# princeton-vl/CER-MVS

Measured on AMD Instinct MI355X. Metric: depth-maps/sec (ref+N src views) at DTU 1600x1184; HBM GB/s vs roofline, higher is better.
Workload: dtype f32 [dense convs: f32 operands split into 2 x f16, f32 accumulate; encoders f16 main term + the two 2^-11 correction terms in e2m3 (FP6, one power-of-two scale per 16-channel block: features 4e-5 from the three-term form), update-block convs f16 main term + the two 2^-11 correction terms in e4m3 on

## Files before the change

### cer-mvs_amd/csrc/conv_s16.hip

```cpp
#include "conv_s16_shared.hpp"
#include "pack.hpp"

struct SxStage {
    int kind;
    const char* base;
    long mtb;
    int g;
};

template <int WM_, int WN_, int MT, int EPI, int F8>
__global__ __launch_bounds__(256, 2) void conv3x3_s16_kernel(const S16Args a) {
    constexpr int TH = WM_ * 2 * MT, HR = TH + 2;
    constexpr int ABUF = HR * (F8 ? SX_ROWB8 : SX_ROWB);
    constexpr int NPIX = HR * SX_HW, NITEM = NPIX * 4, ITEMS = (NITEM + 255) / 256;
    constexpr bool F6 = F8 == 2;
    constexpr int NITEM8 = NPIX * 4, ITEMS8 = F8 ? (NITEM8 + 255) / 256 : 1;
    constexpr int NB = WN_ * 32;
    constexpr int DROWS = HR + 6;
    extern __shared__ __attribute__((aligned(16))) char sx_smem[];
    float* ldsD = reinterpret_cast<float*>(sx_smem + 2 * ABUF);

    const int tid = threadIdx.x, lane = tid & 63, wave = __builtin_amdgcn_readfirstlane(tid >> 6);
    const int wm = wave / WN_, wn = wave % WN_;
    const int li = lane & 31, kg = lane >> 5;
    CER_FUZZ_INIT();
#if SX_TRACE
    unsigned long long trace_t[24];
    int trace_n = 0;
    trace_t[trace_n++] = __builtin_readcyclecounter();
#define SX_STAMP() do { if (trace_n < 24) trace_t[trace_n++] = __builtin_readcyclecounter(); } while (0)
#else
#define SX_STAMP() do { } while (0)
#endif

    auto xcd_order = [](int n, int j) {
        const int q = n >> 3, r = n & 7, xcd = j & 7, k = j >> 3;
        return (xcd < r ? xcd * (q + 1) : r * (q + 1) + (xcd - r) * q) + k;
    };
    int tile, by;
    int tile_y, tile_x;
    if (a.border_first) {
        const int bid = blockIdx.x, tys = a.ntiles / a.tiles_x, nbord = 2 * tys + 2 * (a.tiles_x - 2);
        if (bid < 2 * tys) {
            tile_y = bid >> 1; tile_x = (bid & 1) ? a.tiles_x - 1 : 0;
        } else if (bid < nbord) {
            const int r2 = bid - 2 * tys;
            tile_y = (r2 & 1) ? tys - 1 : 0; tile_x = 1 + (r2 >> 1);
        } else {
            const int i = xcd_order(a.ntiles - nbord, bid - nbord);
            tile_y = 1 + i / (a.tiles_x - 2); tile_x = 1 + i - (tile_y - 1) * (a.tiles_x - 2);
        }
        tile = tile_y * a.tiles_x + tile_x;
        by = 0;
    } else {
        const int vid = xcd_order((int)gridDim.x, (int)blockIdx.x);
        tile = vid / a.ny; by = vid - tile * a.ny;
        tile_y = tile / a.tiles_x; tile_x = tile - tile_y * a.tiles_x;
    }
    const int ty0 = tile_y * TH, tx0 = tile_x * SX_TW;
    const int nb0 = by * NB;
    const int NT = a.cout >> 5;

    int ntens = a.nsrc;
    const float* dsrc = nullptr;
    if (a.kind[a.nsrc - 1] == 1) { ntens = a.nsrc - 1; dsrc = reinterpret_cast<const float*>(a.src[a.nsrc - 1]); }
    const bool interior = ty0 >= 1 && ty0 + TH <= a.h - 1 && tx0 >= 1 && tx0 + SX_TW <= a.w - 1;
    const bool coll = dsrc && a.wpk_c && (interior || a.edge);
    int nsteps = 0;
    for (int s = 0; s < ntens; ++s) nsteps += (a.ch[s] >> 4) * 9;
    const int nsteps_t = nsteps;
    if (dsrc) nsteps += coll ? 6 : 36;
#if SX_STAGGER
    if ((int)gridDim.x > 3 * SX_STAGGER_CUS && (int)blockIdx.x < 2 * SX_STAGGER_CUS) {
        const unsigned hw = __builtin_amdgcn_s_getreg((4 << 0) | (0 << 6) | (31 << 11));
        if ((hw >> SX_STAGGER_BIT) & 1)
            for (int i = 0; i < nsteps * SX_STAGGER; ++i) __builtin_amdgcn_s_sleep(1);
    }
#endif
    const char* wlane = reinterpret_cast<const char*>(coll ? a.wpk_c : a.wpk) + ((long)(nb0 >> 5) + wn) * 2048 + lane * 16;
    const long wstep = (long)NT * 2048;
    const char* wlane8 = reinterpret_cast<const char*>(coll ? a.wpk_c : a.wpk) + ((long)(nb0 >> 5) + wn) * 4096 + lane * 16;

    int xh[3], xl[3];
#pragma unroll
    for (int dx = 0; dx < 3; ++dx) {
        const int col = (li & 15) + dx;
        const int base = (2 * wm * MT + (li >> 4)) * SX_ROWB + col * 64;
        const int sl = kg ^ ((col >> 2) & 3);
        xh[dx] = base + sl * 16;
        xl[dx] = base + (sl ^ 2) * 16;
    }

    int st_pk[ITEMS];
#pragma unroll
    for (int i = 0; i < ITEMS; ++i) {
        const int it = tid + 256 * i;
        const int n = min(it >> 2, NPIX - 1), ps = it & 3;
        const int r = n / SX_HW, c = n - r * SX_HW;
        const int gy = ty0 + r - 1, gx = tx0 + c - 1;
        const bool valid = gy >= 0 && gy < a.h && gx >= 0 && gx < a.w;
        const int cy = min(max(gy, 0), a.h - 1), cx = min(max(gx, 0), a.w - 1);
        const int logical = ps ^ ((c >> 2) & 3);
        st_pk[i] = ((cy >> 1) * a.mtx + (cx >> 4)) | ((((cy & 1) << 4) | (cx & 15)) << 20) | (logical << 25) | ((valid ? 1 : 0) << 27) |
                   ((it < NITEM ? 1 : 0) << 28);
    }
    constexpr int IB = (ITEMS + 1) / 2;
    uint4 raw[IB];
    int vary = 0;
    auto stage_load = [&](const SxStage& st, int batch) {
#pragma unroll
        for (int k = 0; k < IB; ++k) {
            const int i = batch * IB + k;
            if (i >= ITEMS) break;
            const int pk = st_pk[i] ^ vary;
            const char* p = st.base + (long)(pk & 0xFFFFF) * st.mtb + (((pk >> 25) & 3) * 512 + ((pk >> 20) & 31) * 16);
            raw[k] = *reinterpret_cast<const uint4*>(p);
        }
    };
    auto stage_store = [&](int bufoff, int batch) {
        CER_FUZZ_POINT();
        const int tid_ = tid ^ vary;
#pragma unroll
        for (int k = 0; k < IB; ++k) {
            const int i = batch * IB + k;
            if (i >= ITEMS) break;
            const int pk = st_pk[i] ^ vary;
            const unsigned m = (pk & (1 << 27)) ? 0xFFFFFFFFu : 0u;
            uint4 v = raw[k];
            v.x &= m; v.y &= m; v.z &= m; v.w &= m;
            const int it = tid_ + 256 * i;
            const int n = it >> 2, r = n / SX_HW, c = n - r * SX_HW;
            if (pk & (1 << 28)) *reinterpret_cast<uint4*>(sx_smem + bufoff + (r * SX_PITCH + c) * 64 + (it & 3) * 16) = v;
        }
    };
    int xa[3];
    if constexpr (F8) {
#pragma unroll
        for (int dx = 0; dx < 3; ++dx) {
            const int col = (li & 15) + dx;
            xa[dx] = (2 * wm * MT + (li >> 4)) * SX_ROWB8 + col * 128 + (((2 * kg) ^ ((col >> 1) & 7)) << 4);
        }
    }
    int st8_pk[ITEMS8];
    if constexpr (F8) {
#pragma unroll
        for (int i = 0; i < ITEMS8; ++i) {
            const int it = tid + 256 * i;
            const int n = min(it >> 2, NPIX - 1);
            const int r = n / SX_HW, c = n - r * SX_HW;
            const int gy = ty0 + r - 1, gx = tx0 + c - 1;
            const bool valid = gy >= 0 && gy < a.h && gx >= 0 && gx < a.w;
            const int cy = min(max(gy, 0), a.h - 1), cx = min(max(gx, 0), a.w - 1);
            st8_pk[i] = ((cy >> 1) * a.mtx + (cx >> 4)) | ((((cy & 1) << 4) | (cx & 15)) << 20) | ((valid ? 1 : 0) << 28) | ((it < NITEM8 ? 1 : 0) << 29);
        }
    }
    constexpr int IB8 = (ITEMS8 + 2) / 3;
    constexpr int NLD8 = 2;
    uint4 raw8[IB8][NLD8];
    auto stage8_addr = [&](const SxStage& st, int pk, int it) {
        return st.base + (long)(pk & 0xFFFFF) * st.mtb + (((it >> 1) & 1) * 2048 + (it & 1) * 512 + ((pk >> 20) & 31) * 16);
    };
    auto stage6_put = [&](int bufoff, int pk, int it, uint4 vh, uint4 vl) {
        const unsigned m = (pk & (1 << 28)) ? 0xFFFFFFFFu : 0u;
        vh.x &= m; vh.y &= m; vh.z &= m; vh.w &= m;
// ... 98 lines not shown
                const float u[8] = {v[8 * kh], v[8 * kh + 1], v[8 * kh + 2], v[8 * kh + 3], v[8 * kh + 4], v[8 * kh + 5], v[8 * kh + 6], v[8 * kh + 7]};
                half8 hi, lo;
                sx_split8(u, a.disp_scale, hi, lo);
                *reinterpret_cast<half8*>(px + ((kh ^ key) * 16)) = hi;
                SX_LDS_STORE_WAIT();
                *reinterpret_cast<half8*>(px + (((2 + kh) ^ key) * 16)) = lo;
                SX_LDS_STORE_WAIT();
            }
        }
    };
    auto gen_collapsed = [&](int g, int bufoff) {
        auto half_unit = [&](auto kh_tag, int n) {
            constexpr int kh = decltype(kh_tag)::value;
            const int pr = n >> 4, pc = n & 15;
            const float* dp = ldsD + pr * SX_DTW + pc;
            const float ctr = dp[4 * SX_DTW + 4];
            float v[8];
#pragma unroll
            for (int k = 0; k < 8; ++k) {
                const int s = 16 * g + 8 * kh + k;
                const int sy = (s * 57) >> 9, sx = s - 9 * sy;
                v[k] = (s < 81) ? 100.0f * (dp[sy * SX_DTW + sx] - ctr) : 0.f;
            }
            const int c = pc + 1;
            char* px = sx_smem + bufoff + ((pr + 1) * SX_PITCH + c) * 64;
            const int key = (c >> 2) & 3;
            half8 hi, lo;
            sx_split8(v, a.disp_scale, hi, lo);
            *reinterpret_cast<half8*>(px + ((kh ^ key) * 16)) = hi;
            SX_LDS_STORE_WAIT();
            *reinterpret_cast<half8*>(px + (((2 + kh) ^ key) * 16)) = lo;
            SX_LDS_STORE_WAIT();
        };
        CER_FUZZ_POINT();
        for (int u = tid ^ vary; u < TH * SX_TW; u += 256) {
            half_unit(std::integral_constant<int, 0>{}, u);
            half_unit(std::integral_constant<int, 1>{}, u);
        }
    };
    auto stage_tap = [&](const SxStage& st, int bufoff, int t) {
        if (st.kind == 2) {
            if constexpr (F8) {
                if (t == 0) stage8_load(st, 0);
                if (t == 2) { stage8_store(bufoff, 0); stage8_load(st, 1); }
                if (t == 4) { stage8_store(bufoff, 1); stage8_load(st, 2); }
                if (t == 6) stage8_store(bufoff, 2);
            } else {
                if (t == 0) stage_load(st, 0);
                if (t == 3) { stage_store(bufoff, 0); stage_load(st, 1); }
                if (t == 6) stage_store(bufoff, 1);
            }
        } else if (t == 6) {
            if (st.kind == 1) gen_literal(st.g, bufoff);
            else if (st.kind == 3) gen_collapsed(st.g, bufoff);
        }
    };
    auto barrier = [&]() {
        __builtin_amdgcn_fence(__ATOMIC_RELEASE, "workgroup", "local");
        __builtin_amdgcn_s_barrier();
        __builtin_amdgcn_fence(__ATOMIC_ACQUIRE, "workgroup", "local");
        CER_FUZZ_POINT();
    };

    int ngroups_t = 0;
    for (int s = 0; s < ntens; ++s) ngroups_t += a.ch[s] >> (F8 ? 5 : 4);
    const int ngroups = ngroups_t + (dsrc ? (coll ? 6 : 4) : 0);
    auto describe = [&](int gi) {
        SxStage st;
        st.kind = 0; st.base = nullptr; st.mtb = 0; st.g = 0;
        if (gi >= ngroups) return st;
        if (gi >= ngroups_t) { st.kind = coll ? 3 : 1; st.g = gi - ngroups_t; return st; }
        int s = 0, g = gi;
        while (g >= (a.ch[s] >> (F8 ? 5 : 4))) { g -= a.ch[s] >> (F8 ? 5 : 4); ++s; }
        st.kind = 2; st.base = a.src[s] + g * (F8 ? 4096 : 2048); st.mtb = (long)(a.ch[s] >> 4) * 2048;
        return st;
    };

    struct XFrag { half8 h[MT], l[MT]; };
    struct WFrag { half8 h, l; };
    XFrag fx;
    WFrag fw[3];
    auto load_w = [&](WFrag& f, int step) {
        const char* p = wlane + (long)min(step, nsteps - 1) * wstep;
        f.h = *reinterpret_cast<const half8*>(p);
        f.l = *reinterpret_cast<const half8*>(p + 1024);
    };
    const SxStage st0 = describe(0);
    uint4 raw0[F8 ? NLD8 * ITEMS8 : ITEMS];
    if (st0.kind == 2) {
        if constexpr (F8) {
#pragma unroll
            for (int i = 0; i < ITEMS8; ++i) {
                const char* p = stage8_addr(st0, st8_pk[i], tid + 256 * i);
#pragma unroll
                for (int q = 0; q < NLD8; ++q) raw0[NLD8 * i + q] = *reinterpret_cast<const uint4*>(p + 1024 * q);
            }
        } else {
#pragma unroll
            for (int i = 0; i < ITEMS; ++i) {
                const int pk = st_pk[i];
                raw0[i] = *reinterpret_cast<const uint4*>(st0.base + (long)(pk & 0xFFFFF) * st0.mtb + (((pk >> 25) & 3) * 512 + ((pk >> 20) & 31) * 16));
            }
        }
    }
    constexpr int DITEMS = (DROWS * SX_DTW + 255) / 256;
    float dval[DITEMS];
    if (dsrc) {
#pragma unroll
        for (int i = 0; i < DITEMS; ++i) {
            const int idx = tid + 256 * i;
            const int r = idx / SX_DTW, c = idx - r * SX_DTW;
            const int gy = ty0 + r - 4, gx = tx0 + c - 4;
            dval[i] = (idx < DROWS * SX_DTW && gy >= 0 && gy < a.h && gx >= 0 && gx < a.w) ? dsrc[(long)gy * a.w + gx] : 0.f;
        }
    }
    typedef unsigned uintx3 __attribute__((ext_vector_type(3)));
    struct Op8 {
        uint4 a;
        typename std::conditional<F8 == 2, uintx3, uint4>::type b;
        __device__ __forceinline__ void load(const char* p0, const char* p1) {
            a = *reinterpret_cast<const uint4*>(p0);
            b = *reinterpret_cast<const decltype(b)*>(p1);
        }
        __device__ __forceinline__ intx8 v() const {
            if constexpr (F8 == 2) {
                const intx8 lo = (intx8){(int)a.x, (int)a.y, (int)a.z, (int)a.w, (int)b.x, (int)b.y, 0, 0};
                return __builtin_shufflevector(lo, lo, 0, 1, 2, 3, 4, 5, -1, -1);
            } else {
                return (intx8){(int)a.x, (int)a.y, (int)a.z, (int)a.w, (int)b.x, (int)b.y, (int)b.z, (int)b.w};
            }
        }
        __device__ __forceinline__ int scale() const { return (int)b.z; }
    };
    struct W8 { half8 h0, h1; Op8 q; };
    constexpr int WR = (F8 && WM_ == 2 && MT == 2) ? 3 : 2;
    W8 w8[WR];
    auto load_w8 = [&](W8& f, int cstep) {
        const char* p = wlane8 + (long)min(cstep, (nsteps_t >> 1) - 1) * (2 * wstep);
        f.h0 = *reinterpret_cast<const half8*>(p);
        f.h1 = *reinterpret_cast<const half8*>(p + 1024);
        f.q.load(p + 2048, p + 3072);
    };
    if (F8 && ngroups_t > 0) {
        load_w8(w8[0], 0);
        if constexpr (WR == 3) load_w8(w8[1], 1);
    } else {
        load_w(fw[0], 0);
        load_w(fw[1], 1);
    }
    const int mrow0 = (ty0 >> 1) + wm * MT;
    const long mt0 = (long)mrow0 * a.mtx + tile_x;
    floatx16 acc[MT];
#pragma unroll
    for (int m = 0; m < MT; ++m) {
        const bool ok = mrow0 + m < a.mty;
#pragma unroll
        for (int j = 0; j < 4; ++j) {
            float4 v = make_float4(0.f, 0.f, 0.f, 0.f);
            if (a.init) {
                if (ok) v = cer_ld4(reinterpret_cast<const float*>(reinterpret_cast<const char*>(a.init) +
                                                                     (((mt0 + (long)m * a.mtx) * NT + (nb0 >> 5) + wn) * 4 + j) * 1024 + lane * 16));
            } else if (a.bias) {
                v = cer_ld4(a.bias + nb0 + wn * 32 + 8 * j + 4 * kg);
            }
            acc[m][4 * j + 0] = v.x; acc[m][4 * j + 1] = v.y; acc[m][4 * j + 2] = v.z; acc[m][4 * j + 3] = v.w;
        }
    }
    if (dsrc) {
#pragma unroll
        for (int i = 0; i < DITEMS; ++i)
            if (tid + 256 * i < DROWS * SX_DTW) ldsD[tid + 256 * i] = dval[i];
    }
    if (st0.kind == 2) {
        if constexpr (F8) {
#pragma unroll
            for (int i = 0; i < ITEMS8; ++i) {
                if constexpr (F6) stage6_put(0, st8_pk[i], tid + 256 * i, raw0[2 * i], raw0[2 * i + 1]);
                else stage8_put(0, st8_pk[i], tid + 256 * i, raw0[2 * i], raw0[2 * i + 1]);
            }
        } else {
#pragma unroll
            for (int i = 0; i < ITEMS; ++i) {
                const int pk = st_pk[i];
                const unsigned m = (pk & (1 << 27)) ? 0xFFFFFFFFu : 0u;
                uint4 v = raw0[i];
                v.x &= m; v.y &= m; v.z &= m; v.w &= m;
                const int it = tid + 256 * i;
                const int n = it >> 2, r = n / SX_HW, c = n - r * SX_HW;
                if (pk & (1 << 28)) *reinterpret_cast<uint4*>(sx_smem + (r * SX_PITCH + c) * 64 + (it & 3) * 16) = v;
            }
        }
    } else {
        barrier();
        stage_tap(st0, 0, 6);
    }
    barrier();
#pragma unroll
    for (int m = 0; m < MT; ++m)
#pragma unroll
        for (int r = 0; r < 16; ++r) acc[m][r] *= a.S;

    auto load_x = [&](XFrag& f, int ph, int pl, int rowoff) {
#pragma unroll
        for (int m = 0; m < MT; ++m) {
            f.h[m] = *reinterpret_cast<const half8*>(sx_smem + ph + (2 * m) * SX_ROWB + rowoff);
            f.l[m] = *reinterpret_cast<const half8*>(sx_smem + pl + (2 * m) * SX_ROWB + rowoff);
        }
    };
    auto mma_roll = [&](const WFrag& w, int ph, int pl, int rowoff) {
#pragma unroll
        for (int m = 0; m < MT; ++m) acc[m] = __builtin_amdgcn_mfma_f32_32x32x16_f16(w.h, fx.h[m], acc[m], 0, 0, 0);
#pragma unroll
        for (int m = 0; m < MT; ++m) {
            acc[m] = __builtin_amdgcn_mfma_f32_32x32x16_f16(w.l, fx.h[m], acc[m], 0, 0, 0);
            fx.h[m] = *reinterpret_cast<const half8*>(sx_smem + ph + (2 * m) * SX_ROWB + rowoff);
            __builtin_amdgcn_sched_barrier(0);
        }
#pragma unroll
        for (int m = 0; m < MT; ++m) {
            acc[m] = __builtin_amdgcn_mfma_f32_32x32x16_f16(w.h, fx.l[m], acc[m], 0, 0, 0);
            fx.l[m] = *reinterpret_cast<const half8*>(sx_smem + pl + (2 * m) * SX_ROWB + rowoff);
            __builtin_amdgcn_sched_barrier(0);
        }
    };

    const bool first_is_centre0 = st0.kind == 3;
    typedef Op8 F8Frag;
    F8Frag f8[F8 ? MT : 1];
    if (F8 && st0.kind == 2) {
#pragma unroll
        for (int m = 0; m < MT; ++m) {
            fx.h[m] = *reinterpret_cast<const half8*>(sx_smem + xa[0] + (2 * m) * SX_ROWB8);
            fx.l[m] = *reinterpret_cast<const half8*>(sx_smem + (xa[0] ^ 16) + (2 * m) * SX_ROWB8);
            f8[m].load(sx_smem + (xa[0] ^ 64) + (2 * m) * SX_ROWB8, sx_smem + (xa[0] ^ 80) + (2 * m) * SX_ROWB8);
        }
    } else if (first_is_centre0) load_x(fx, xh[1], xl[1], SX_ROWB);
    else load_x(fx, xh[0], xl[0], 0);

    SX_STAMP();
    int step = 0, gi = 0;
    if constexpr (F8) {
        auto mma_corr = [&](const W8& w, const F8Frag& x, const floatx16& c) {
            if constexpr (F6) return __builtin_amdgcn_mfma_scale_f32_32x32x64_f8f6f4(w.q.v(), x.v(), c, 2, 2, 0, w.q.scale(), 0, x.scale());
            else return __builtin_amdgcn_mfma_scale_f32_32x32x64_f8f6f4(w.q.v(), x.v(), c, 0, 0, 0, 127, 0, 130);
        };
        auto mma8_roll = [&](W8& w, int pa, int rowoff) {
#pragma unroll
            for (int m = 0; m < MT; ++m) acc[m] = __builtin_amdgcn_mfma_f32_32x32x16_f16(w.h0, fx.h[m], acc[m], 0, 0, 0);
#pragma unroll
            for (int m = 0; m < MT; ++m) {
                acc[m] = __builtin_amdgcn_mfma_f32_32x32x16_f16(w.h1, fx.l[m], acc[m], 0, 0, 0);
                fx.h[m] = *reinterpret_cast<const half8*>(sx_smem + pa + (2 * m) * SX_ROWB8 + rowoff);
                __builtin_amdgcn_sched_barrier(0);
            }
#pragma unroll
            for (int m = 0; m < MT; ++m) {
                acc[m] = mma_corr(w, f8[m], acc[m]);
                fx.l[m] = *reinterpret_cast<const half8*>(sx_smem + (pa ^ 16) + (2 * m) * SX_ROWB8 + rowoff);
                f8[m].load(sx_smem + (pa ^ 64) + (2 * m) * SX_ROWB8 + rowoff, sx_smem + (pa ^ 80) + (2 * m) * SX_ROWB8 + rowoff);
                __builtin_amdgcn_sched_barrier(0);
            }
        };
        auto mma8_last = [&](W8& w, int ph, int pl, int rowoff) {
#pragma unroll
            for (int m = 0; m < MT; ++m) acc[m] = __builtin_amdgcn_mfma_f32_32x32x16_f16(w.h0, fx.h[m], acc[m], 0, 0, 0);
#pragma unroll
            for (int m = 0; m < MT; ++m) {
                acc[m] = __builtin_amdgcn_mfma_f32_32x32x16_f16(w.h1, fx.l[m], acc[m], 0, 0, 0);
                fx.h[m] = *reinterpret_cast<const half8*>(sx_smem + ph + (2 * m) * SX_ROWB + rowoff);
                __builtin_amdgcn_sched_barrier(0);
            }
#pragma unroll
            for (int m = 0; m < MT; ++m) {
                acc[m] = mma_corr(w, f8[m], acc[m]);
                fx.l[m] = *reinterpret_cast<const half8*>(sx_smem + pl + (2 * m) * SX_ROWB + rowoff);
                __builtin_amdgcn_sched_barrier(0);
            }
        };
        auto chunk = [&](auto last_tag) {
            constexpr bool last = decltype(last_tag)::value;
            vary = (gi >> 28) * 0x11111111;
            const SxStage nx = describe(gi + 1);
            const int bufC = (gi & 1) * ABUF, bufN = ABUF - bufC;
#pragma unroll
            for (int t = 0; t < 9; ++t) {
                if (nx.kind == 2 ? (t == 0 || t == 2 || t == 4 || t == 6) : t == 6) stage_tap(nx, bufN, t);
                if (t == 8) barrier();
                W8& wc = w8[WR == 3 ? t % 3 : (t & 1)];
                W8& wn = w8[WR == 3 ? (t + 2) % 3 : ((t + 1) & 1)];
                if (WR == 3 ? (t < 7 || !last) : (t < 8 || !last)) load_w8(wn, gi * 9 + t + WR - 1);
                if (t == 8 && last) { load_w(fw[0], nsteps_t); load_w(fw[1], nsteps_t + 1); }
                __builtin_amdgcn_sched_barrier(0);
                if (t < 8) mma8_roll(wc, (xa[(t + 1) % 3] ^ vary) + bufC, ((t + 1) / 3) * SX_ROWB8);
                else if (!last) mma8_roll(wc, (xa[0] ^ vary) + bufN, 0);
                else mma8_last(wc, xh[1] + bufN, xl[1] + bufN, SX_ROWB);
            }
            if constexpr (WR == 2) {
                if (!last) {
                    const W8 tmp = w8[0]; w8[0] = w8[1]; w8[1] = tmp;
                }
            }
            SX_STAMP();
            ++gi;
        };
        while (gi + 1 < ngroups_t) chunk(std::false_type{});
        if (gi < ngroups_t) chunk(std::true_type{});
        step = nsteps_t;
    }
    const int ngroups9 = F8 ? 0 : ngroups_t + ((dsrc && !coll) ? 4 : 0);
    for (; gi < ngroups9; ++gi, step += 9) {
        vary = (gi >> 28) * 0x11111111;
        const SxStage nx = describe(gi + 1);
        const int bufC = (gi & 1) * ABUF, bufN = ABUF - bufC;
        const bool nxt_centre = nx.kind == 3;
#pragma unroll
        for (int t = 0; t < 9; ++t) {
            if (t == 0 || t == 3 || t == 6) stage_tap(nx, bufN, t);
            if (t == 8) barrier();
            load_w(fw[(t + 2) % 3], step + t + 2);
            __builtin_amdgcn_sched_barrier(0);
            if (t < 8) mma_roll(fw[t % 3], xh[(t + 1) % 3] + bufC, xl[(t + 1) % 3] + bufC, ((t + 1) / 3) * SX_ROWB);
            else if (nxt_centre) mma_roll(fw[t % 3], xh[1] + bufN, xl[1] + bufN, SX_ROWB);
            else mma_roll(fw[t % 3], xh[0] + bufN, xl[0] + bufN, 0);
        }
        SX_STAMP();
    }
    if (dsrc && coll) {
        vary = (gi >> 28) * 0x11111111;
#pragma unroll
        for (int t = 0; t < 6; ++t) {
            const int bufC = ((gi + t) & 1) * ABUF, bufN = ABUF - bufC;
            if (t < 5) {
                gen_collapsed(t + 1, bufN);
                barrier();
            }
            load_w(fw[(t + 2) % 3], step + t + 2);
            __builtin_amdgcn_sched_barrier(0);
            mma_roll(fw[t % 3], xh[1] + bufN, xl[1] + bufN, SX_ROWB);
        }
        step += 6;
        gi += 6;
    }
    SX_STAMP();

    if (coll && a.edge && !interior) {
        const _Float16* ew = reinterpret_cast<const _Float16*>(a.edge) + ((long)(nb0 >> 5) + wn) * 1024 + lane * 8;
#pragma unroll
        for (int m = 0; m < MT; ++m) {
            const int py = 2 * (wm * MT + m) + (li >> 4), px = li & 15;
            const int y = ty0 + py, x = tx0 + px;
            const bool in = y < a.h && x < a.w;
            const bool top = in && y == 0, bot = in && y == a.h - 1, lef = in && x == 0, rig = in && x == a.w - 1;
            auto D = [&](int r, int c) { return ldsD[(r - ty0 + 4) * SX_DTW + (c - tx0 + 4)]; };
            auto apply = [&](int e, int nks, bool on, auto&& pos) {
                if (!__any(on)) return;
#pragma unroll
                for (int ks = 0; ks < 2; ++ks) {
                    if (ks >= nks) break;
                    float v[8];
#pragma unroll
                    for (int q = 0; q < 8; ++q) {
                        const int k = 16 * ks + 8 * kg + q;
                        int r = 0, c = 0;
                        const bool ok = pos(k, r, c);
                        v[q] = (on && ok) ? 100.0f * D(r, c) : 0.f;
                    }
                    half8 fh, fl;
                    sx_split8(v, a.disp_scale, fh, fl);
                    const _Float16* wp = ew + (long)((e * 2 + ks) * NT) * 1024;
                    const half8 wh = *reinterpret_cast<const half8*>(wp), wl = *reinterpret_cast<const half8*>(wp + 512);
                    acc[m] = __builtin_amdgcn_mfma_f32_32x32x16_f16(wh, fh, acc[m], 0, 0, 0);
                    acc[m] = __builtin_amdgcn_mfma_f32_32x32x16_f16(wh, fl, acc[m], 0, 0, 0);
                    acc[m] = __builtin_amdgcn_mfma_f32_32x32x16_f16(wl, fh, acc[m], 0, 0, 0);
                }
            };
            apply(0, 2, top, [&](int k, int& r, int& c) { r = k / 9; c = x + k % 9 - 4; return k < 27; });
            apply(1, 2, bot, [&](int k, int& r, int& c) { r = a.h - 3 + k / 9; c = x + k % 9 - 4; return k < 27; });
            apply(2, 2, lef, [&](int k, int& r, int& c) { r = y + k / 3 - 4; c = k % 3; return k < 27; });
            apply(3, 2, rig, [&](int k, int& r, int& c) { r = y + k / 3 - 4; c = a.w - 3 + k % 3; return k < 27; });
            apply(4, 1, top && lef, [&](int k, int& r, int& c) { r = k / 3; c = k % 3; return k < 9; });
            apply(5, 1, top && rig, [&](int k, int& r, int& c) { r = k / 3; c = a.w - 3 + k % 3; return k < 9; });
            apply(6, 1, bot && lef, [&](int k, int& r, int& c) { r = a.h - 3 + k / 3; c = k % 3; return k < 9; });
            apply(7, 1, bot && rig, [&](int k, int& r, int& c) { r = a.h - 3 + k / 3; c = a.w - 3 + k % 3; return k < 9; });
        }
    }
    const int half = a.cout >> 1;
    if constexpr (EPI == SX_EPI_DELTA) {
        static_assert(EPI != SX_EPI_DELTA || WM_ == 1, "the DELTA epilogue is built for the 1 x 4 wave layout");
        const _Float16* w2 = reinterpret_cast<const _Float16*>(a.aux) + ((long)(by * WN_ + wn) * 2) * 1024;
        float* red = reinterpret_cast<float*>(sx_smem);
        static_assert(WN_ * MT * 9 * 32 * 4 <= 2 * ABUF, "reduction scratch does not fit");
        barrier();
        const float hs = a.invS * (float)(1 << SX_HID_LOG2);
        float hmax = 0.f;
#pragma unroll
        for (int m = 0; m < MT; ++m) {
            floatx16 tm;
#pragma unroll
            for (int r = 0; r < 16; ++r) tm[r] = 0.f;
#pragma unroll
            for (int jp = 0; jp < 2; ++jp) {
                float v[8];
#pragma unroll
                for (int e = 0; e < 4; ++e) {
                    const auto sw = __builtin_amdgcn_permlane32_swap(__float_as_uint(acc[m][8 * jp + e]), __float_as_uint(acc[m][8 * jp + 4 + e]), false, false);
                    v[e] = fmaxf(__uint_as_float(sw[0]), 0.f);
                    v[4 + e] = fmaxf(__uint_as_float(sw[1]), 0.f);
                }
                hmax = fmaxf(hmax, fmaxf(fmaxf(fmaxf(v[0], v[1]), fmaxf(v[2], v[3])), fmaxf(fmaxf(v[4], v[5]), fmaxf(v[6], v[7]))));
                half8 hh, hl;
                sx_split8(v, hs, hh, hl);
                const half8 wh = *reinterpret_cast<const half8*>(w2 + (jp * 2 + 0) * 512 + lane * 8);
                const half8 wl = *reinterpret_cast<const half8*>(w2 + (jp * 2 + 1) * 512 + lane * 8);
                tm = __builtin_amdgcn_mfma_f32_32x32x16_f16(wh, hh, tm, 0, 0, 0);
                tm = __builtin_amdgcn_mfma_f32_32x32x16_f16(wh, hl, tm, 0, 0, 0);
                tm = __builtin_amdgcn_mfma_f32_32x32x16_f16(wl, hh, tm, 0, 0, 0);
            }
            float* rp = red + ((wn * MT + m) * 9) * 32 + li;
#pragma unroll
            for (int r = 0; r < 4; ++r) rp[(r + 4 * kg) * 32] = tm[r];
            if (kg == 0) rp[8 * 32] = tm[4];
        }
        if (a.flag && __ballot(!(hmax * hs <= 65504.0f)) != 0ull && lane == 0) atomicOr(a.flag, 2);
        barrier();
        const long P = (long)a.h * a.w;
        for (int idx = tid; idx < MT * 9 * 32; idx += 256) {
            const int m = idx / (9 * 32), rem = idx - m * 9 * 32, tap = rem >> 5, px = rem & 31;
            float s = 0.f;
#pragma unroll
            for (int q = 0; q < WN_; ++q) s += red[((q * MT + m) * 9 + tap) * 32 + px];
            const int gy = ty0 + 2 * m + (px >> 4), gx = tx0 + (px & 15);
            if (gy < a.h && gx < a.w) a.out[((long)by * 9 + tap) * P + (long)gy * a.w + gx] = s * a.proj_inv;
        }
        return;
    } else {
        const int nt = (nb0 >> 5) + wn;
        auto piece = [&](int m, int G, int g) { return (((mt0 + (long)m * a.mtx) * G + g) * 2) * 1024 + lane * 16; };
        if (EPI == CER_EPI_LINEAR && !a.out_split) {
#pragma unroll
            for (int m = 0; m < MT; ++m) {
                if (mrow0 + m >= a.mty) continue;
#pragma unroll
                for (int j = 0; j < 4; ++j)
                    *reinterpret_cast<float4*>(reinterpret_cast<char*>(a.out) + (((mt0 + (long)m * a.mtx) * NT + nt) * 4 + j) * 1024 + lane * 16) =
                        make_float4(acc[m][4 * j] * a.invS, acc[m][4 * j + 1] * a.invS, acc[m][4 * j + 2] * a.invS, acc[m][4 * j + 3] * a.invS);
            }
        } else {
            const bool is_r = EPI == CER_EPI_GATES && nt * 32 >= half;
            const int G = (EPI == CER_EPI_GATES ? half : a.cout) >> 4;
            const int g0 = (EPI == CER_EPI_GATES ? ((nt * 32) % half) >> 4 : nt * 2);
            half8 ph[MT][2], pl[MT][2];
            float4 z0[MT][2], z1[MT][2];
            if ((EPI == CER_EPI_GATES && is_r) || EPI == CER_EPI_GRU) {
#pragma unroll
                for (int m = 0; m < MT; ++m)
#pragma unroll
                    for (int jp = 0; jp < 2; ++jp) {
                        if (mrow0 + m >= a.mty) continue;
                        const char* p = reinterpret_cast<const char*>(a.aux) + piece(m, G, g0 + jp);
                        ph[m][jp] = *reinterpret_cast<const half8*>(p);
                        pl[m][jp] = *reinterpret_cast<const half8*>(p + 1024);
                        if (EPI == CER_EPI_GRU) {
                            const char* zp = reinterpret_cast<const char*>(a.aux2) + piece(m, G, g0 + jp);
                            z0[m][jp] = *reinterpret_cast<const float4*>(zp);
                            z1[m][jp] = *reinterpret_cast<const float4*>(zp + 1024);
                        }
                    }
            }
#pragma unroll
            for (int m = 0; m < MT; ++m) {
#pragma unroll
                for (int jp = 0; jp < 2; ++jp) {
                    float v[8];
#pragma unroll
                    for (int e = 0; e < 4; ++e) {
                        const auto sw = __builtin_amdgcn_permlane32_swap(__float_as_uint(acc[m][8 * jp + e]), __float_as_uint(acc[m][8 * jp + 4 + e]), false, false);
                        v[e] = __uint_as_float(sw[0]) * a.invS;
                        v[4 + e] = __uint_as_float(sw[1]) * a.invS;
                    }
                    if (mrow0 + m >= a.mty) continue;
                    const long off = piece(m, G, g0 + jp);
                    auto st_split = [&](float* base, const float (&o)[8]) {
                        half8 hi, lo;
                        sx_split8(o, a.out_scale, hi, lo);
                        *reinterpret_cast<half8*>(reinterpret_cast<char*>(base) + off) = hi;
                        *reinterpret_cast<half8*>(reinterpret_cast<char*>(base) + off + 1024) = lo;
                    };
                    if (EPI == CER_EPI_LINEAR || EPI == CER_EPI_RELU) {
                        if (EPI == CER_EPI_RELU)
#pragma unroll
                            for (int e = 0; e < 8; ++e) v[e] = fmaxf(v[e], 0.f);
                        st_split(a.out, v);
                    } else if (EPI == CER_EPI_GATES) {
#pragma unroll
                        for (int e = 0; e < 8; ++e) v[e] = sx_sigmoid(v[e]);
                        if (!is_r) {
                            *reinterpret_cast<float4*>(reinterpret_cast<char*>(a.out) + off) = make_float4(v[0], v[1], v[2], v[3]);
                            *reinterpret_cast<float4*>(reinterpret_cast<char*>(a.out) + off + 1024) = make_float4(v[4], v[5], v[6], v[7]);
                        } else {
                            float hp[8];
                            sx_join8(ph[m][jp], pl[m][jp], a.aux_inv, hp);
#pragma unroll
                            for (int e = 0; e < 8; ++e) v[e] *= hp[e];
                            st_split(a.out2, v);
                        }
                    } else if (EPI == CER_EPI_GRU) {
                        float hp[8];
                        sx_join8(ph[m][jp], pl[m][jp], a.aux_inv, hp);
                        const float z[8] = {z0[m][jp].x, z0[m][jp].y, z0[m][jp].z, z0[m][jp].w, z1[m][jp].x, z1[m][jp].y, z1[m][jp].z, z1[m][jp].w};
#pragma unroll
                        for (int e = 0; e < 8; ++e) v[e] = (1.0f - z[e]) * hp[e] + z[e] * sx_tanh(v[e]);
                        st_split(a.out, v);
                    }
                }
            }
        }
    }
#if SX_TRACE
    if ((EPI == CER_EPI_GATES || EPI == CER_EPI_GRU) && lane == 0) {
        unsigned long long* tb = (unsigned long long*)(EPI == CER_EPI_GATES ? (const void*)a.aux2 : (const void*)a.out2) + ((long)blockIdx.x * 4 + wave) * 32;
        tb[0] = (unsigned long long)trace_n;
        tb[1] = __builtin_amdgcn_s_getreg((4 << 0) | (0 << 6) | (31 << 11));
        tb[2] = __builtin_amdgcn_s_getreg((20 << 0) | (0 << 6) | (31 << 11));
        tb[3] = __builtin_readcyclecounter();
        tb[4] = (unsigned long long)nsteps;
#pragma unroll
        for (int k = 0; k < 24; ++k) tb[8 + k] = trace_t[k];
    }
#endif
}


template <int WM_, int WN_, int MT, int F8>
static int sx_launch(S16Args& a, int epi, hipStream_t st) {
    constexpr int TH = WM_ * 2 * MT, HR = TH + 2;
    const size_t smem = 2 * HR * (F8 ? SX_ROWB8 : SX_ROWB) + (HR + 6) * SX_DTW * 4;
    const int tiles_y = (a.h + TH - 1) / TH;
    a.tiles_x = (a.w + SX_TW - 1) / SX_TW;
    a.mtx = a.tiles_x;
    a.mty = (a.h + 1) / 2;
    if ((long)a.mtx * a.mty >= (1L << 20)) return CER_ESHAPE;
    a.ntiles = a.tiles_x * tiles_y;
    a.ny = a.cout / (WN_ * 32);
    a.border_first = a.edge && a.wpk_c && a.nsrc > 0 && a.kind[a.nsrc - 1] == 1 && a.ny == 1 && a.tiles_x >= 3 && tiles_y >= 3;
    dim3 grid((unsigned)(a.ntiles * a.ny)), block(256);
    if (smem > 64 * 1024) {
        static bool raised[64][5];
        int dev_ = 0;
        if (hipGetDevice(&dev_) != hipSuccess || dev_ < 0 || dev_ >= 64) dev_ = 0;
        const void* fn = nullptr;
        switch (epi) {
            case CER_EPI_LINEAR: fn = (const void*)conv3x3_s16_kernel<WM_, WN_, MT, CER_EPI_LINEAR, F8>; break;
            case CER_EPI_RELU: fn = (const void*)conv3x3_s16_kernel<WM_, WN_, MT, CER_EPI_RELU, F8>; break;
            case CER_EPI_GRU: fn = (const void*)conv3x3_s16_kernel<WM_, WN_, MT, CER_EPI_GRU, F8>; break;
            default: break;
        }
        if constexpr (WM_ == 1) {
            if (epi == CER_EPI_GATES) fn = (const void*)conv3x3_s16_kernel<WM_, WN_, MT, CER_EPI_GATES, F8>;
            if (epi == SX_EPI_DELTA) fn = (const void*)conv3x3_s16_kernel<WM_, WN_, MT, SX_EPI_DELTA, F8>;
        }
        if (!fn || epi < 0 || epi > 4) return CER_EINVAL;
        if (!raised[dev_][epi]) {
            if (hipFuncSetAttribute(fn, hipFuncAttributeMaxDynamicSharedMemorySize, (int)smem) != hipSuccess) return CER_EINVAL;
            raised[dev_][epi] = true;
        }
    }
    switch (epi) {
        case CER_EPI_LINEAR: hipLaunchKernelGGL((conv3x3_s16_kernel<WM_, WN_, MT, CER_EPI_LINEAR, F8>), grid, block, smem, st, a); break;
        case CER_EPI_RELU: hipLaunchKernelGGL((conv3x3_s16_kernel<WM_, WN_, MT, CER_EPI_RELU, F8>), grid, block, smem, st, a); break;
        case CER_EPI_GRU: hipLaunchKernelGGL((conv3x3_s16_kernel<WM_, WN_, MT, CER_EPI_GRU, F8>), grid, block, smem, st, a); break;
        case CER_EPI_GATES:
            if constexpr (WM_ == 1) {
                hipLaunchKernelGGL((conv3x3_s16_kernel<WM_, WN_, MT, CER_EPI_GATES, F8>), grid, block, smem, st, a);
                break;
            } else {
                return CER_ESHAPE;
            }
        case SX_EPI_DELTA:
            if constexpr (WM_ == 1) {
                hipLaunchKernelGGL((conv3x3_s16_kernel<WM_, WN_, MT, SX_EPI_DELTA, F8>), grid, block, smem, st, a);
                break;
            } else {
                return CER_ESHAPE;
            }
        default: return CER_EINVAL;
    }
    CER_RETURN_IF_LAUNCH_FAILED();
    return CER_OK;
}

static int sx_num_cus() { return cer_num_cus(); }

extern "C" int cer_conv3x3_s16(const cer_conv_inputs* in, const int* log2sx, const void* packed_w, const void* packed_collapsed,
                               const void* edge_w, int log2S, const float* bias, const float* init, float* out, float* out2, const float* aux, const float* aux2, int h,
                               int w, int Cout, int epi, int log2s_out, int log2s_aux, int tile_mt, void* stream) {
    if (!in || !log2sx || !packed_w || !out || h <= 0 || w <= 0 || Cout <= 0) return CER_EINVAL;
    if (in->nsrc <= 0 || in->nsrc > CER_CONV_MAX_SRC) return CER_EINVAL;
    const int out_split = (epi & CER_EPI_OUT_SPLIT) != 0;
    const int corr_fp6 = (epi & CER_EPI_CORR_FP6) != 0;
    const int corr_fp8 = (epi & CER_EPI_CORR_FP8) != 0 || corr_fp6;
    if ((epi & CER_EPI_CORR_FP8) && corr_fp6) return CER_EINVAL;
    epi &= ~(CER_EPI_OUT_SPLIT | CER_EPI_AUX_SPLIT | CER_EPI_CORR_FP8 | CER_EPI_CORR_FP6);
    if (epi == CER_EPI_GATES && (!out2 || !aux || Cout != 128)) return CER_EINVAL;
    if (epi == CER_EPI_GRU && (!aux || !aux2)) return CER_EINVAL;
    if (epi == SX_EPI_DELTA && (!aux || Cout % 128 != 0)) return CER_EINVAL;
    if (Cout % 64 != 0) return CER_ESHAPE;
    if ((long)h * w >= (1L << 27)) return CER_ESHAPE;
    if (!cer_aligned16(packed_w) || !cer_aligned16(packed_collapsed) || !cer_aligned16(edge_w) || !cer_aligned16(init) || !cer_aligned16(bias) || !cer_aligned16(out) ||
        !cer_aligned16(out2) || !cer_aligned16(aux) || !cer_aligned16(aux2))
        return CER_EALIGN;
    S16Args a;
    memset(&a, 0, sizeof(a));
    int order[CER_CONV_MAX_SRC];
    const int nd = sx_order(in->kind, in->nsrc, order);
    if (nd > 1) return CER_ESHAPE;
    a.nsrc = in->nsrc;
    for (int oi = 0; oi < in->nsrc; ++oi) {
        const int s = order[oi];
        if (!in->src[s]) return CER_EINVAL;
        if (in->kind[s] != 1 && in->kind[s] != 2) return CER_EINVAL;
        if (in->kind[s] == 2 && (in->ch[s] % 32 != 0 || !cer_aligned16(in->src[s]))) return CER_ESHAPE;
        if (in->kind[s] == 1 && in->ch[s] != 49) return CER_ESHAPE;
        a.src[oi] = reinterpret_cast<const char*>(in->src[s]);
        a.ch[oi] = in->ch[s];
        a.kind[oi] = in->kind[s];
        if (in->kind[s] == 1) a.disp_scale = ldexpf(1.0f, log2sx[s]);
    }
    a.wpk = (const _Float16*)packed_w;
    a.wpk_c = (const _Float16*)packed_collapsed;
    a.edge = packed_collapsed ? edge_w : nullptr;
    a.bias = bias;
    a.init = init;
    a.out = out;
    a.out2 = out2;
    a.aux = aux;
    a.aux2 = aux2;
    a.h = h;
    a.w = w;
    a.cout = Cout;
    a.S = ldexpf(1.0f, log2S);
    a.invS = ldexpf(1.0f, -log2S);
    a.out_scale = ldexpf(1.0f, log2s_out);
    a.aux_inv = ldexpf(1.0f, -log2s_aux);
    a.proj_inv = ldexpf(1.0f, -(SX_HID_LOG2 + log2s_aux));
    a.out_split = out_split;
    a.flag = cer_overflow_flag_get();
    hipStream_t st = (hipStream_t)stream;
    const int ncu = sx_num_cus();
    const long slots = 2L * ncu;
    const int tx = (w + SX_TW - 1) / SX_TW;
    auto pick = [&](int rows_per_mt, int lo, int hi, int ny) {
        int best_mt = hi;
        double best = -1.0;
        for (int c = hi; c >= lo; --c) {
            const long nblk = (long)((h + rows_per_mt * c - 1) / (rows_per_mt * c)) * tx * ny;
            const double cost = (double)((nblk + slots - 1) / slots) * (c + 1.1);
            if (best < 0 || cost < best - 1e-9) { best = cost; best_mt = c; }
        }
        return best_mt;
    };
    if (corr_fp8 && nd == 1 && !(packed_collapsed && edge_w)) return CER_ESHAPE;
#if CER_WITH_SXPC
    if (corr_fp8 && tile_mt == 0) {
        S16Args b = a;
        const int rc = sxpc_dispatch(b, epi, tile_mt, st);
        if (rc != CER_ESHAPE) return rc;
    }
#endif
    if (Cout % 128 == 0) {
        int mt = tile_mt;
        if (mt != 2 && mt != 4) mt = pick(2, 2, 4, Cout / 128) == 2 ? 2 : 4;
        if (corr_fp6) return mt == 2 ? sx_launch<1, 4, 2, 2>(a, epi, st) : sx_launch<1, 4, 4, 2>(a, epi, st);
        if (corr_fp8) return mt == 2 ? sx_launch<1, 4, 2, 1>(a, epi, st) : sx_launch<1, 4, 4, 1>(a, epi, st);
        return mt == 2 ? sx_launch<1, 4, 2, 0>(a, epi, st) : sx_launch<1, 4, 4, 0>(a, epi, st);
    }
    if (epi == SX_EPI_DELTA || epi == CER_EPI_GATES) return CER_ESHAPE;
    int mt = tile_mt;
    if (corr_fp8) {
        if (mt < 2 || mt > 3) mt = pick(4, 2, 3, Cout / 64);
        if (corr_fp6) return mt == 2 ? sx_launch<2, 2, 2, 2>(a, epi, st) : sx_launch<2, 2, 3, 2>(a, epi, st);
        return mt == 2 ? sx_launch<2, 2, 2, 1>(a, epi, st) : sx_launch<2, 2, 3, 1>(a, epi, st);
    }
    if (mt < 2 || mt > 4) mt = pick(4, 2, 4, Cout / 64);
    return mt == 2 ? sx_launch<2, 2, 2, 0>(a, epi, st) : mt == 3 ? sx_launch<2, 2, 3, 0>(a, epi, st) : sx_launch<2, 2, 4, 0>(a, epi, st);
}

__global__ __launch_bounds__(256) void s16_layout_kernel(const float* __restrict__ src, float* __restrict__ dst, int w, int C, int layout,
                                                         float scale, float inv, int inverse, int y0, int nrows) {
    const long i = (long)blockIdx.x * 256 + threadIdx.x;
    const long n8 = (long)nrows * w * (C / 8);
    if (i >= n8) return;
    const long pix = i / (C / 8);
    const int cb = (int)(i - pix * (C / 8)) * 8;
    const int y = y0 + (int)(pix / w), x = (int)(pix % w);
    const long mt = (long)(y >> 1) * ((w + 15) >> 4) + (x >> 4);
    const int li = ((y & 1) << 4) | (x & 15);
    char* t = reinterpret_cast<char*>(inverse ? const_cast<float*>(src) : dst);
    float* plain = (inverse ? dst : const_cast<float*>(src)) + pix * C + cb;
    char *p0, *p1;
    if (layout == 0 || layout == 3) {
        p0 = t + ((mt * (C >> 4) + (cb >> 4)) * 2) * 1024 + ((((cb >> 3) & 1) << 5) | li) * 16;
        p1 = p0 + 1024;
    } else if (layout == 1) {
        p0 = t + ((mt * (C >> 5) + (cb >> 5)) * 4 + ((cb & 31) >> 3)) * 1024 + li * 16;
        p1 = p0 + 512;
    } else {
        p0 = t + ((mt * (C >> 4) + (cb >> 4)) * 2) * 1024 + ((((cb >> 3) & 1) << 5) | li) * 16;
        p1 = p0 + 1024;
    }
    float v[8];
    if (!inverse) {
        const float4 t0 = cer_ld4(plain), t1 = cer_ld4(plain + 4);
        v[0] = t0.x; v[1] = t0.y; v[2] = t0.z; v[3] = t0.w; v[4] = t1.x; v[5] = t1.y; v[6] = t1.z; v[7] = t1.w;
        if (layout == 0) {
            half8 hi, lo;
            sx_split8(v, scale, hi, lo);
            *reinterpret_cast<half8*>(p0) = hi;
            *reinterpret_cast<half8*>(p1) = lo;
        } else {
            *reinterpret_cast<float4*>(p0) = t0;
            *reinterpret_cast<float4*>(p1) = t1;
        }
    } else {
        if (layout == 0) {
            sx_join8(*reinterpret_cast<const half8*>(p0), *reinterpret_cast<const half8*>(p1), inv, v);
            *reinterpret_cast<float4*>(plain) = make_float4(v[0], v[1], v[2], v[3]);
            *reinterpret_cast<float4*>(plain + 4) = make_float4(v[4], v[5], v[6], v[7]);
        } else {
            *reinterpret_cast<float4*>(plain) = *reinterpret_cast<const float4*>(p0);
            *reinterpret_cast<float4*>(plain + 4) = *reinterpret_cast<const float4*>(p1);
        }
// ... 50 lines not shown
```

### cer-mvs_amd/csrc/conv_s16_shared.hpp

```cpp
#pragma once
#include "common.hpp"
#include <math.h>
#include <type_traits>
#include <stdlib.h>
#include <string.h>

typedef _Float16 half8 __attribute__((ext_vector_type(8)));
typedef float floatx16 __attribute__((ext_vector_type(16)));
typedef int intx8 __attribute__((ext_vector_type(8)));

#define SX_TW 16
#define SX_HW 18
#define SX_PITCH 20
#define SX_ROWB (SX_PITCH * 64)
#define SX_ROWB8 (SX_PITCH * 128)
#define SX_DTW 24
#define SX_EPI_DELTA 4
#define SX_HID_LOG2 4
#define SX_LDS_STORE_WAIT() asm volatile("s_nop 3" ::: "memory")
#ifndef SX_STAGGER
#define SX_STAGGER 4
#endif
#define SX_STAGGER_BIT 16
#define SX_STAGGER_CUS 256
#ifndef SX_TRACE
#define SX_TRACE 0
#endif

struct S16Args {
    const char* src[CER_CONV_MAX_SRC];
    int ch[CER_CONV_MAX_SRC];
    int kind[CER_CONV_MAX_SRC];
    int nsrc;
    const _Float16* wpk;
    const _Float16* wpk_c;
    const float* bias;
    const float* init;
    float* out;
    float* out2;
    const float* aux;
    const float* aux2;
    const void* edge;
    int h, w, cout, tiles_x, ntiles, ny, mtx, mty;
    int border_first;
    float S, invS;
    float out_scale;
    float aux_inv;
    float disp_scale;
    float proj_inv;
    int out_split;
    int* flag;
};

__device__ __forceinline__ void sx_split8(const float (&v)[8], float scale, half8& hi, half8& lo) {
    cer_h2 h[4], l[4];
#pragma unroll
    for (int i = 0; i < 4; ++i) {
        cer_f2 x = (cer_f2){v[2 * i], v[2 * i + 1]} * scale;
        x = __builtin_elementwise_min(__builtin_elementwise_max(x, (cer_f2){-65504.0f, -65504.0f}), (cer_f2){65504.0f, 65504.0f});
        h[i] = __builtin_convertvector(x, cer_h2);
        l[i] = __builtin_convertvector(x - __builtin_convertvector(h[i], cer_f2), cer_h2);
    }
    hi = (half8){h[0].x, h[0].y, h[1].x, h[1].y, h[2].x, h[2].y, h[3].x, h[3].y};
    lo = (half8){l[0].x, l[0].y, l[1].x, l[1].y, l[2].x, l[2].y, l[3].x, l[3].y};
}
__device__ __forceinline__ void sx_join8(const half8 hi, const half8 lo, float inv, float (&v)[8]) {
#pragma unroll
    for (int e = 0; e < 8; ++e) v[e] = ((float)hi[e] + (float)lo[e]) * inv;
}
__device__ __forceinline__ float sx_sigmoid(float x) { return __builtin_amdgcn_rcpf(1.0f + __builtin_amdgcn_exp2f(-1.4426950408889634f * x)); }
__device__ __forceinline__ float sx_tanh(float x) { return 1.0f - 2.0f * __builtin_amdgcn_rcpf(1.0f + __builtin_amdgcn_exp2f(2.8853900817779268f * x)); }


#ifndef CER_WITH_SXPC
#define CER_WITH_SXPC 0
#endif
int sxpc_dispatch(S16Args& a, int epi, int tile_mt, hipStream_t st);
```

Measured before the change: 74.86.

## Tune s16 conv kernel: runtime stagger CU count, 3-deep weight ring, lane offsets

```diff
diff --git a/cer-mvs_amd/csrc/conv_s16.hip b/cer-mvs_amd/csrc/conv_s16.hip
--- a/cer-mvs_amd/csrc/conv_s16.hip
+++ b/cer-mvs_amd/csrc/conv_s16.hip
@@ -71,15 +71,16 @@
     const int nsteps_t = nsteps;
     if (dsrc) nsteps += coll ? 6 : 36;
 #if SX_STAGGER
-    if ((int)gridDim.x > 3 * SX_STAGGER_CUS && (int)blockIdx.x < 2 * SX_STAGGER_CUS) {
+    if (a.stagger_cus > 0 && (int)gridDim.x > 3 * a.stagger_cus && (int)blockIdx.x < 2 * a.stagger_cus) {
         const unsigned hw = __builtin_amdgcn_s_getreg((4 << 0) | (0 << 6) | (31 << 11));
         if ((hw >> SX_STAGGER_BIT) & 1)
             for (int i = 0; i < nsteps * SX_STAGGER; ++i) __builtin_amdgcn_s_sleep(1);
     }
 #endif
-    const char* wlane = reinterpret_cast<const char*>(coll ? a.wpk_c : a.wpk) + ((long)(nb0 >> 5) + wn) * 2048 + lane * 16;
+    const char* wlane = reinterpret_cast<const char*>(coll ? a.wpk_c : a.wpk) + ((long)(nb0 >> 5) + wn) * 2048;
+    const unsigned lane16 = lane * 16;
     const long wstep = (long)NT * 2048;
-    const char* wlane8 = reinterpret_cast<const char*>(coll ? a.wpk_c : a.wpk) + ((long)(nb0 >> 5) + wn) * 4096 + lane * 16;
+    const char* wlane8 = reinterpret_cast<const char*>(coll ? a.wpk_c : a.wpk) + ((long)(nb0 >> 5) + wn) * 4096;
 
     int xh[3], xl[3];
 #pragma unroll
@@ -344,8 +345,8 @@
     WFrag fw[3];
     auto load_w = [&](WFrag& f, int step) {
         const char* p = wlane + (long)min(step, nsteps - 1) * wstep;
-        f.h = *reinterpret_cast<const half8*>(p);
-        f.l = *reinterpret_cast<const half8*>(p + 1024);
+        f.h = *reinterpret_cast<const half8*>(p + lane16);
+        f.l = *reinterpret_cast<const half8*>(p + lane16 + 1024);
     };
     const SxStage st0 = describe(0);
     uint4 raw0[F8 ? NLD8 * ITEMS8 : ITEMS];
@@ -395,17 +396,19 @@
         __device__ __forceinline__ int scale() const { return (int)b.z; }
     };
     struct W8 { half8 h0, h1; Op8 q; };
-    constexpr int WR = (F8 && WM_ == 2 && MT == 2) ? 3 : 2;
+    constexpr int WR = (F8 && ((WM_ == 2 && MT == 2) || (WM_ == 1 && MT == 4))) ? 3 : 2;
     W8 w8[WR];
     auto load_w8 = [&](W8& f, int cstep) {
         const char* p = wlane8 + (long)min(cstep, (nsteps_t >> 1) - 1) * (2 * wstep);
-        f.h0 = *reinterpret_cast<const half8*>(p);
-        f.h1 = *reinterpret_cast<const half8*>(p + 1024);
-        f.q.load(p + 2048, p + 3072);
-    };
-    if (F8 && ngroups_t > 0) {
-        load_w8(w8[0], 0);
-        if constexpr (WR == 3) load_w8(w8[1], 1);
+        f.h0 = *reinterpret_cast<const half8*>(p + lane16);
+        f.h1 = *reinterpret_cast<const half8*>(p + lane16 + 1024);
+        f.q.load(p + lane16 + 2048, p + lane16 + 3072);
+    };
+    if constexpr (F8) {
+        if (ngroups_t > 0) {
+            load_w8(w8[0], 0);
+            if constexpr (WR == 3) load_w8(w8[1], 1);
+        }
     } else {
         load_w(fw[0], 0);
         load_w(fw[1], 1);
@@ -506,6 +509,12 @@
             if constexpr (F6) return __builtin_amdgcn_mfma_scale_f32_32x32x64_f8f6f4(w.q.v(), x.v(), c, 2, 2, 0, w.q.scale(), 0, x.scale());
             else return __builtin_amdgcn_mfma_scale_f32_32x32x64_f8f6f4(w.q.v(), x.v(), c, 0, 0, 0, 127, 0, 130);
         };
+        auto pin_acc = [&]() {
+            if constexpr (WR == 3 && WM_ == 1) {
+#pragma unroll
+                for (int m = 0; m < MT; ++m) asm volatile("" : "+v"(acc[m]));
+            }
+        };
         auto mma8_roll = [&](W8& w, int pa, int rowoff) {
 #pragma unroll
             for (int m = 0; m < MT; ++m) acc[m] = __builtin_amdgcn_mfma_f32_32x32x16_f16(w.h0, fx.h[m], acc[m], 0, 0, 0);
@@ -522,6 +531,7 @@
                 f8[m].load(sx_smem + (pa ^ 64) + (2 * m) * SX_ROWB8 + rowoff, sx_smem + (pa ^ 80) + (2 * m) * SX_ROWB8 + rowoff);
                 __builtin_amdgcn_sched_barrier(0);
             }
+            pin_acc();
         };
         auto mma8_last = [&](W8& w, int ph, int pl, int rowoff) {
 #pragma unroll
@@ -538,14 +548,15 @@
                 fx.l[m] = *reinterpret_cast<const half8*>(sx_smem + pl + (2 * m) * SX_ROWB + rowoff);
                 __builtin_amdgcn_sched_barrier(0);
             }
+            pin_acc();
         };
         auto chunk = [&](auto last_tag) {
             constexpr bool last = decltype(last_tag)::value;
             vary = (gi >> 28) * 0x11111111;
             const SxStage nx = describe(gi + 1);
             const int bufC = (gi & 1) * ABUF, bufN = ABUF - bufC;
-#pragma unroll
-            for (int t = 0; t < 9; ++t) {
+            auto tap = [&](auto t_tag) {
+                constexpr int t = decltype(t_tag)::value;
                 if (nx.kind == 2 ? (t == 0 || t == 2 || t == 4 || t == 6) : t == 6) stage_tap(nx, bufN, t);
                 if (t == 8) barrier();
                 W8& wc = w8[WR == 3 ? t % 3 : (t & 1)];
@@ -556,7 +567,11 @@
                 if (t < 8) mma8_roll(wc, (xa[(t + 1) % 3] ^ vary) + bufC, ((t + 1) / 3) * SX_ROWB8);
                 else if (!last) mma8_roll(wc, (xa[0] ^ vary) + bufN, 0);
                 else mma8_last(wc, xh[1] + bufN, xl[1] + bufN, SX_ROWB);
-            }
+            };
+            auto taps = [&](auto... ts) { (tap(ts), ...); };
+            taps(std::integral_constant<int, 0>{}, std::integral_constant<int, 1>{}, std::integral_constant<int, 2>{}, std::integral_constant<int, 3>{},
+                 std::integral_constant<int, 4>{}, std::integral_constant<int, 5>{}, std::integral_constant<int, 6>{}, std::integral_constant<int, 7>{},
+                 std::integral_constant<int, 8>{});
             if constexpr (WR == 2) {
                 if (!last) {
                     const W8 tmp = w8[0]; w8[0] = w8[1]; w8[1] = tmp;
@@ -567,6 +582,7 @@
         };
         while (gi + 1 < ngroups_t) chunk(std::false_type{});
         if (gi < ngroups_t) chunk(std::true_type{});
+        else { load_w(fw[0], 0); load_w(fw[1], 1); }
         step = nsteps_t;
     }
     const int ngroups9 = F8 ? 0 : ngroups_t + ((dsrc && !coll) ? 4 : 0);
@@ -604,6 +620,19 @@
         gi += 6;
     }
     SX_STAMP();
+#if SX_TRACE
+    auto trace_out = [&](const void* buf) {
+        if (lane != 0) return;
+        unsigned long long* tb = (unsigned long long*)buf + ((long)blockIdx.x * 4 + wave) * 32;
+        tb[0] = (unsigned long long)trace_n;
+        tb[1] = __builtin_amdgcn_s_getreg((4 << 0) | (0 << 6) | (31 << 11));
+        tb[2] = __builtin_amdgcn_s_getreg((20 << 0) | (0 << 6) | (31 << 11));
+        tb[3] = __builtin_readcyclecounter();
+        tb[4] = (unsigned long long)nsteps;
+#pragma unroll
+        for (int k = 0; k < 24; ++k) tb[8 + k] = trace_t[k];
+    };
+#endif
 
     if (coll && a.edge && !interior) {
         const _Float16* ew = reinterpret_cast<const _Float16*>(a.edge) + ((long)(nb0 >> 5) + wn) * 1024 + lane * 8;
@@ -694,6 +723,9 @@
             const int gy = ty0 + 2 * m + (px >> 4), gx = tx0 + (px & 15);
             if (gy < a.h && gx < a.w) a.out[((long)by * 9 + tap) * P + (long)gy * a.w + gx] = s * a.proj_inv;
         }
+#if SX_TRACE
+        if (a.aux2) trace_out(a.aux2);
+#endif
         return;
     } else {
         const int nt = (nb0 >> 5) + wn;
@@ -779,16 +811,7 @@
         }
     }
 #if SX_TRACE
-    if ((EPI == CER_EPI_GATES || EPI == CER_EPI_GRU) && lane == 0) {
-        unsigned long long* tb = (unsigned long long*)(EPI == CER_EPI_GATES ? (const void*)a.aux2 : (const void*)a.out2) + ((long)blockIdx.x * 4 + wave) * 32;
-        tb[0] = (unsigned long long)trace_n;
-        tb[1] = __builtin_amdgcn_s_getreg((4 << 0) | (0 << 6) | (31 << 11));
-        tb[2] = __builtin_amdgcn_s_getreg((20 << 0) | (0 << 6) | (31 << 11));
-        tb[3] = __builtin_readcyclecounter();
-        tb[4] = (unsigned long long)nsteps;
-#pragma unroll
-        for (int k = 0; k < 24; ++k) tb[8 + k] = trace_t[k];
-    }
+    if (EPI == CER_EPI_GATES || EPI == CER_EPI_GRU) trace_out(EPI == CER_EPI_GATES ? (const void*)a.aux2 : (const void*)a.out2);
 #endif
 }
 
@@ -909,6 +932,7 @@
     a.flag = cer_overflow_flag_get();
     hipStream_t st = (hipStream_t)stream;
     const int ncu = sx_num_cus();
+    a.stagger_cus = ncu > 0 ? ncu : 0;
     const long slots = 2L * ncu;
     const int tx = (w + SX_TW - 1) / SX_TW;
     auto pick = [&](int rows_per_mt, int lo, int hi, int ny) {
diff --git a/cer-mvs_amd/csrc/conv_s16_shared.hpp b/cer-mvs_amd/csrc/conv_s16_shared.hpp
--- a/cer-mvs_amd/csrc/conv_s16_shared.hpp
+++ b/cer-mvs_amd/csrc/conv_s16_shared.hpp
@@ -22,7 +22,6 @@
 #define SX_STAGGER 4
 #endif
 #define SX_STAGGER_BIT 16
-#define SX_STAGGER_CUS 256
 #ifndef SX_TRACE
 #define SX_TRACE 0
 #endif
@@ -43,6 +42,7 @@
     const void* edge;
     int h, w, cout, tiles_x, ntiles, ny, mtx, mty;
     int border_first;
+    int stagger_cus;
     float S, invS;
     float out_scale;
     float aux_inv;
```

Result: no change. 74.85 (-0.0%).
